# robustrobotics/multi_view_stereonet

Hardware: AMD Instinct MI355X
Metric: depthmaps/sec at 512x256, 64 hypotheses, 2 src views; L1 vs ref (higher is better)
Workload: dtype f32; 1 GPU; GTA-SfM-shaped 512x256, D=64 hypotheses, 2 source views, cost-volume filter + 5 refiners; global_batch=256, parallelism=dp1 (independent images, all-gather of metric rows)

## Files before the change

multi_view_stereonet_amd/csrc/mvsn_conv_wino.hip:

```cpp
#include <type_traits>
#include <utility>

#include "mvsn_resident.h"
#include "mvsn_conv_wino.h"

namespace mvsn {

constexpr int WN_THREADS = 512, WN_WAVES = 8;
constexpr int WN_TY = 16, WN_TX = 32;
constexpr int WN_WIDE_TY = 10, WN_WIDE_TX = 40, WN_WIDE_PC = WN_WIDE_TX / 2, WN_WIDE_NP = (WN_WIDE_TY / 2) * WN_WIDE_PC;
constexpr int WN_ROLL_PR = 6, WN_ROLL_NP = WN_ROLL_PR * WN_WIDE_PC, WN_ROLL_HY = 2 * WN_ROLL_PR + 3;
constexpr int WN_TILE_RP = 3;
constexpr int wn_pa(int dil) { return (dil + 3) / 4 * 4; }
constexpr int WN_UFLOATS = 16 * 128;
constexpr int WN_MAX_CHUNKS = 9;
constexpr int WN_LDS_MAX = 160 * 1024;

__device__ floatx4 g_wn_zero16 = {0.f, 0.f, 0.f, 0.f};

#ifndef MVSN_WN_ABLATE
#define MVSN_WN_ABLATE 0
#endif

#ifndef MVSN_RD_ABLATE
// ... 86 lines not shown
    {2, 4, 1, true, 0, 2, false, 24},
    {2, 3, 1, true, 1, 2, false, 24},
};
constexpr int WN_NFORMS = sizeof(WN_FORMS) / sizeof(WN_FORMS[0]);
constexpr int wn_find_form(const WinoForm &f, int from = 0) {
  for (int i = from; i < WN_NFORMS; ++i)
    if (WN_FORMS[i].same(f)) return i;
  return -1;
}
constexpr bool wn_forms_ok() {
  for (int i = 0; i < WN_NFORMS; ++i)
    if (WN_FORMS[i].bytes(WN_FORMS[i].chunks) > WN_LDS_MAX || wn_find_form(WN_FORMS[i], i + 1) >= 0) return false;
  return true;
}
static_assert(wn_forms_ok(), "a kernel form needs more than 160 KB of LDS, or is listed twice");

template <bool LDSONLY>
__device__ __forceinline__ void wn_barrier() {
  if constexpr (LDSONLY) asm volatile("s_waitcnt lgkmcnt(0)\n\ts_barrier" ::: "memory");
  else __syncthreads();
}

#pragma clang diagnostic push
#pragma clang diagnostic ignored "-Winline-asm"
template <bool ASM>
__device__ __forceinline__ void wn_dma16(const float *g, const float *l) {
  if constexpr (ASM) {
    const unsigned la = __builtin_amdgcn_readfirstlane((unsigned)(size_t)MVSN_LPTR(l));
    asm volatile("s_mov_b32 m0, %1\n\ts_nop 0\n\tglobal_load_lds_dwordx4 %0, off" ::"v"(g), "s"(la) : "memory", "m0");
  } else {
    __builtin_amdgcn_global_load_lds(MVSN_GPTR(g), MVSN_LPTR(l), 16, 0, 0);
  }
}
template <bool ASM>
__device__ __forceinline__ void wn_dma16_buf(const float *base, unsigned bytes, unsigned voff, const float *l) {
  if constexpr (ASM) {
    typedef int wn_srd_t __attribute__((ext_vector_type(4)));
    const size_t b = (size_t)base;
    wn_srd_t srd;
    srd[0] = __builtin_amdgcn_readfirstlane((int)(unsigned)b);
    srd[1] = __builtin_amdgcn_readfirstlane((int)((unsigned)(b >> 32) & 0xFFFFu));
    srd[2] = __builtin_amdgcn_readfirstlane((int)bytes);
    srd[3] = 0x00020000;
    const unsigned la = __builtin_amdgcn_readfirstlane((unsigned)(size_t)MVSN_LPTR(l));
#if MVSN_WN_NT_RAW
    asm volatile("s_mov_b32 m0, %2\n\ts_nop 0\n\tbuffer_load_dwordx4 %0, %1, 0 offen nt lds" ::"v"(voff), "s"(srd), "s"(la)
                 : "memory", "m0");
#else
    asm volatile("s_mov_b32 m0, %2\n\ts_nop 0\n\tbuffer_load_dwordx4 %0, %1, 0 offen lds" ::"v"(voff), "s"(srd), "s"(la)
                 : "memory", "m0");
#endif
  } else {
    __builtin_amdgcn_raw_ptr_buffer_load_lds(__builtin_amdgcn_make_buffer_rsrc(const_cast<float *>(base), 0, (int)bytes, 0x00020000),
                                             MVSN_LPTR(l), 16, (int)voff, 0, 0, MVSN_WN_NT_RAW ? 2 : 0);
  }
}
#pragma clang diagnostic pop

typedef unsigned wn_uintx2 __attribute__((ext_vector_type(2)));
typedef unsigned wn_uintx4 __attribute__((ext_vector_type(4)));
__device__ __forceinline__ __amdgpu_buffer_rsrc_t wn_rsrc(const void *base, unsigned bytes) {
  return __builtin_amdgcn_make_buffer_rsrc(const_cast<void *>(base), 0, (int)bytes, 0x00020000);
}
template <int AUX>
__device__ __forceinline__ void wn_store2(__amdgpu_buffer_rsrc_t r, unsigned voff, unsigned soff, float a, float b) {
  wn_uintx2 d;
  d[0] = __builtin_bit_cast(unsigned, a), d[1] = __builtin_bit_cast(unsigned, b);
  __builtin_amdgcn_raw_buffer_store_b64(d, r, (int)voff, (int)soff, AUX);
}
template <int AUX>
__device__ __forceinline__ void wn_store4(__amdgpu_buffer_rsrc_t r, unsigned voff, unsigned soff, floatx4 v) {
  __builtin_amdgcn_raw_buffer_store_b128(__builtin_bit_cast(wn_uintx4, v), r, (int)voff, (int)soff, AUX);
}

struct WinoDiv {
  unsigned mul, shift;
};
static WinoDiv wino_div(unsigned d) {
  unsigned s = 0;
  while ((1u << s) < d) ++s;
  const unsigned long long m = ((1ull << 32) * ((1ull << s) - d)) / d + 1;
  return WinoDiv{(unsigned)m, s};
}
__device__ __forceinline__ int wdiv(int n, WinoDiv f) { return (int)((__umulhi((unsigned)n, f.mul) + (unsigned)n) >> f.shift); }

struct WinoArgs {
  int n, cin, H, W, ntx, tiles, nchunks;
  WinoDiv fd_ntx;
  int cb0, cb1;
  const float *in1, *in2;
  size_t bs0, cs0;
  int rev;
  int D;
  int pr;
  WinoDiv fd_pr;
  int nty, rpy;
};

struct RideArgs {
  const float *x, *stats, *gamma, *beta;
  const float *res, *r_stats, *r_gamma, *r_beta;
  float *out;
  int units;
  WinoDiv fd_upp;
};
typedef const __attribute__((address_space(4))) float *wn_cfloat;
__device__ __forceinline__ float wn_sload(const float *p, size_t i) { return ((wn_cfloat)(size_t)p)[i]; }

__global__ void wino_pack_kernel(const float *__restrict__ w, int cin, int cout, int nchunks, int kd,
                                 float *__restrict__ out) {
  const int total = nchunks * WN_UFLOATS;
  const int idx = blockIdx.x * blockDim.x + threadIdx.x;
  if (idx >= total) return;
  const int lane = idx & 63, t = (idx >> 6) & 1, xi = (idx >> 7) & 15, chunk = idx >> 11;
  const int per_kz = nchunks / kd, kz = chunk / per_kz;
  const int co = t * 16 + (lane & 15), ci = (chunk - kz * per_kz) * 4 + (lane >> 4);
  float u = 0.0f;
  if (co < cout && ci < cin) {
    const float *g = w + (((size_t)co * cin + ci) * kd + kz) * 9;
    const float G[4][3] = {{1.f, 0.f, 0.f}, {0.5f, 0.5f, 0.5f}, {0.5f, -0.5f, 0.5f}, {0.f, 0.f, 1.f}};
    const int i = xi >> 2, j = xi & 3;
    for (int a = 0; a < 3; ++a)
      for (int b = 0; b < 3; ++b) u += G[i][a] * g[a * 3 + b] * G[j][b];
  }
  out[idx] = u;
}

#ifndef MVSN_WN_NO_FULLW
#define MVSN_WN_FULLW_OK 1
#else
#define MVSN_WN_FULLW_OK 0
#endif
template <int MODE, int KS, int NSTAGE, int DIL, bool VOL = false, int RIDE = 0, int TILE = 0, bool FULLW = false>
__global__ __launch_bounds__(WN_THREADS, 2) void conv_wino_kernel(WinoArgs g, const float *__restrict__ in,
                                                                  const float *__restrict__ upk,
                                                                  const float *__restrict__ bias,
                                                                  const float *__restrict__ in_stats,
                                                                  const float *__restrict__ in_gamma,
                                                                  const float *__restrict__ in_beta,
                                                                  float *__restrict__ out,
                                                                  float *__restrict__ out_partials, RideArgs rd,
                                                                  MVSN_VIS10) {
  extern __shared__ __attribute__((aligned(16))) float smem[];
#ifdef MVSN_WN_FORCE_DMA
  constexpr bool ASM_DMA = MVSN_WN_FORCE_DMA;
#else
  constexpr bool ASM_DMA = RIDE > 0 && DIL == 1;
#endif
#ifdef MVSN_WN_FORCE_BARRIER
  constexpr bool LDS_BARRIER = MVSN_WN_FORCE_BARRIER;
#else
  constexpr bool LDS_BARRIER = !VOL;
#endif
  constexpr bool RP = TILE == WN_TILE_RP;
  constexpr int WIDE = RP ? 0 : TILE;
  static_assert(!WIDE || (VOL && DIL == 1 && MVSN_WN_TRANSPOSED), "wide tiles: volume form only (transposed epilogue)");
  constexpr bool ROLL = WIDE == 2;
  constexpr int TY = ROLL ? 2 * WN_ROLL_PR : (WIDE ? WN_WIDE_TY : WN_TY), TX = WIDE ? WN_WIDE_TX : WN_TX;
  static_assert(!RP || (DIL > 1 && !VOL && !WIDE), "row-phase items: dilated 2-D layers");
  constexpr WinoForm L{KS, NSTAGE, DIL, VOL, RIDE, TILE, FULLW};
  constexpr int HY = L.hy(), XS = L.xs();
  constexpr int VS = RP ? 1 : DIL;
  constexpr int YS = RP ? DIL : 1;
  auto item_y0 = [](int tq) { return RP ? (tq & (DIL - 1)) + (int)((unsigned)tq / DIL) * (TY * DIL) : tq * TY; };
  constexpr int NP = ROLL ? WN_ROLL_NP : WN_WIDE_NP;
  constexpr int PA = wn_pa(DIL), DQ = XS / 4, GROUPS = HY * DQ, PIECES = (GROUPS + 63) / 64;
  static_assert(XS == TX + 2 * PA && HY == (ROLL ? WN_ROLL_HY : TY + 2 * VS), "the LDS plan's raw tile is this kernel's tile plus its halo");
  constexpr int RCST = L.rcst(), STAGE = L.stage();
  float *U = smem + L.u();
  static_assert(!FULLW || (DIL == 1 && WIDE == 0 && MVSN_WN_XF == 2 && MVSN_WN_TRANSPOSED), "full-width form: 16 x 32 tiles, burst + block");
  constexpr int SHIFT = (DIL == 1 && MVSN_WN_SHIFT && !FULLW) ? 1 : 0;
  constexpr int CSHIFT = (DIL > 1 && MVSN_WN_SHIFT) ? DIL : 0;
  constexpr int UST = KS * WN_UFLOATS;
  constexpr bool TR = DIL == 1 && MVSN_WN_TRANSPOSED;
  static_assert(!VOL || (KS == 2 && DIL == 1), "volume form: 32 channels in steps of 8, dilation 1");
  const int nsteps = (g.nchunks + KS - 1) / KS;
  const int uchunks = VOL ? NSTAGE * KS : nsteps * KS;

  const int tid = threadIdx.x, lane = tid & 63;
  const int wave = __builtin_amdgcn_readfirstlane(tid >> 6);
  const size_t plane = (size_t)g.H * g.W;
  const int ptiles = ROLL ? g.tiles : (RP ? DIL * g.rpy * g.ntx : g.D * g.tiles);
  auto roll_item = [&](int t, int &zA, int &prA0, int &sA) {
    const int R0 = t * WN_ROLL_PR;
    zA = wdiv(R0, g.fd_pr);
    prA0 = R0 - zA * g.pr;
    sA = g.pr - prA0 < WN_ROLL_PR ? g.pr - prA0 : WN_ROLL_PR;
  };
  const int total = g.n * ptiles;
  const int G = gridDim.x;
  const int slot = xcd_tile_index(blockIdx.x, G);
#ifdef MVSN_WN_STAMPS
  unsigned long long *dbg = (blockIdx.x == gridDim.x / 3 && tid == 0) ? g_wn_stamps : nullptr;
  unsigned long long *dbg_lds = reinterpret_cast<unsigned long long *>(U + L.stamps(uchunks));
  int dbg_i = 0;
  bool dbg_on = true;
#endif
  WN_STAMP();

  if constexpr (!VOL) {
    const int runs = g.nchunks * (WN_UFLOATS / 256);
    for (int run = wave; run < runs; run += WN_WAVES)
      wn_dma16<ASM_DMA>(upk + (size_t)run * 256 + lane * 4, U + run * 256);
    if (uchunks != g.nchunks)
      *reinterpret_cast<floatx4 *>(U + g.nchunks * WN_UFLOATS + tid * 4) = floatx4{0.f, 0.f, 0.f, 0.f};
  }

  float *bias_lds = U + L.bias(uchunks);
  if (tid < 32) bias_lds[tid] = bias ? bias[tid] : 0.0f;

  constexpr int STEP_PIECES = KS * 4 * PIECES;
  constexpr bool EVEN = STEP_PIECES % WN_WAVES == 0;
  constexpr int PER = EVEN ? STEP_PIECES / WN_WAVES : 2;
  static_assert(EVEN || (KS == 1 && PIECES == 3), "uneven DMA split only for the 12-piece case");
  static_assert(!EVEN || PIECES % PER == 0 || PER % PIECES == 0, "a wave's pieces stay within one channel");
  const int dch = EVEN ? (wave * PER) / PIECES : (wave & 3);
  const int dp0 = EVEN ? (wave * PER) % PIECES : (wave < 4 ? 0 : 2);
  const int dpn = EVEN ? (PER < PIECES ? PER : PIECES) : (wave < 4 ? 2 : 1);
  const float *zero = reinterpret_cast<const float *>(&g_wn_zero16);
  int pf_round = 0, pf_chunk = 0, pf_stage = 0;
  int pf_goff[PER];
  int pf_n = 0, pf_z = 0;
  bool pf_live = slot < total;
  int rd_young = 0;
  auto pf_plan = [&]() {
    const int flat = g.rev ? total - 1 - (pf_round * G + slot) : pf_round * G + slot;
    const int n = flat / ptiles;
    int tile = flat - n * ptiles;
    int r_pr0 = 0, r_s = WN_ROLL_PR;
    if constexpr (ROLL) {
      roll_item(tile, pf_z, r_pr0, r_s);
      tile = 0;
    } else if constexpr (VOL) {
      pf_z = tile / g.tiles;
      tile -= pf_z * g.tiles;
    }
    const int tyi = ROLL ? 0 : wdiv(tile, g.fd_ntx), txi = tile - tyi * g.ntx;
    const int y0 = ROLL ? 2 * r_pr0 : item_y0(tyi), x0 = txi * TX;
    pf_n = n;
    int lo;
    asm volatile("v_mbcnt_lo_u32_b32 %0, -1, 0\n\tv_mbcnt_hi_u32_b32 %0, -1, %0" : "=v"(lo));
#pragma unroll
    for (int i = 0; i < PER; ++i) {
      const int e = (dp0 + i) * 64 + lo;
      const int row = e / DQ, q = e - row * DQ;
      int gy = y0 - DIL + YS * row;
      const int gx = x0 - PA + 4 * q;
      int zsh = 0;
      if constexpr (ROLL) {
        const bool isb = (r_s < WN_ROLL_PR) & (row >= 2 * r_s + 1);
        gy = isb ? row - (2 * r_s + 2) : gy;
        zsh = isb ? g.H * g.W : 0;
      }
      const bool ok = (i < dpn) & (e < GROUPS) & (gy >= 0) & (gy < g.H) & (gx >= 0) & (gx < g.W);
      pf_goff[i] = ok ? (zsh + gy * g.W + gx) * (MVSN_WN_BUFDMA ? 4 : 1) : -1;
    }
  };
  auto pf_issue = [&]() {
    if (!pf_live) return;
    rd_young += PER;
    bool cok;
    const float *src;
    unsigned rbytes = 0;
    bool roll_first = false;
    if constexpr (ROLL) {
      const int kz = pf_chunk >> 2, c = (pf_chunk & 3) * 8 + dch, zz = pf_z + kz - 1;
      cok = zz >= 0 && zz < g.D;
      roll_first = zz < 0;
      const int zlo = zz < 0 ? 0 : zz, zhi = zz + 1 < g.D ? zz + 1 : g.D - 1;
      const int np = zhi - zlo + 1 > 0 ? zhi - zlo + 1 : 0;
      const int zsel = zlo < g.D - 1 ? zlo : g.D - 1;
      src = in + (size_t)(unsigned)__builtin_amdgcn_readfirstlane((pf_n * 32 + c) * g.D + zsel) * plane;
      rbytes = (unsigned)np * (unsigned)plane * 4u;
      rbytes = (unsigned)__builtin_amdgcn_readfirstlane((int)rbytes);
    } else if constexpr (VOL) {
      const int kz = pf_chunk >> 2, c = (pf_chunk & 3) * 8 + dch, zz = pf_z + kz - 1;
      cok = zz >= 0 && zz < g.D;
      src = in + (((size_t)pf_n * 32 + c) * g.D + (cok ? zz : 0)) * plane;
    } else {
      const int c = pf_chunk * (KS * 4) + dch;
      cok = c < g.cin;
      const int cc = cok ? c : 0, c1 = cc - g.cb0, c2 = c1 - g.cb1;
      src = c1 < 0 ? in + (size_t)pf_n * g.bs0 + (size_t)cc * g.cs0
          : c2 < 0 ? g.in1 + ((size_t)pf_n * g.cb1 + c1) * plane
                   : g.in2 + ((size_t)pf_n * (g.cin - g.cb0 - g.cb1) + c2) * plane;
    }
    float *dst = smem + pf_stage * STAGE + dch * RCST + SHIFT + CSHIFT * (dch & 1);
    const unsigned pbytes = ROLL ? rbytes : (cok ? (unsigned)plane * 4u : 0u);
#pragma unroll
    for (int i = 0; i < PER; ++i) {
      if (i < dpn) {
        if ((dp0 + i) * 64 + lane < GROUPS) {
          if constexpr (ROLL) {
            static_assert(!ROLL || MVSN_WN_BUFDMA, "rolling strips: descriptor DMA only");
            unsigned off = (unsigned)pf_goff[i];
            off -= roll_first ? (unsigned)plane * 4u : 0u;
            wn_dma16_buf<ASM_DMA>(src, pbytes, off, dst + (dp0 + i) * 256);
          } else if constexpr (MVSN_WN_BUFDMA) {
            wn_dma16_buf<ASM_DMA>(src, pbytes, (unsigned)pf_goff[i], dst + (dp0 + i) * 256);
          } else {
            const float *p = (cok && pf_goff[i] >= 0) ? src + pf_goff[i] : zero;
            wn_dma16<ASM_DMA>(p, dst + (dp0 + i) * 256);
          }
        }
      }
    }
// ... 107 lines not shown
            else xf_mask |= 1u << i;
          }
        }
      }
      int c = xf_chunk * (KS * 4) + dch;
      bool live = c < g.cin;
      if constexpr (VOL) {
        const int zz = z + (xf_chunk >> 2) - 1;
        c = (xf_chunk & 3) * 8 + dch;
        live = zz >= 0 && zz < g.D;
        if constexpr (ROLL) {
          const bool liveb = zz + 1 < g.D;
          xf_mask = (live ? xf_maska : 0u) | (liveb ? xf_maskb : 0u);
          live = live || liveb;
        }
      }
      if (live) {
        const float mean = in_stats[((size_t)n * 4 + (c >> 3)) * 2 + 0];
        const float rstd = in_stats[((size_t)n * 4 + (c >> 3)) * 2 + 1];
        xf_sc = rstd * in_gamma[c];
        xf_sh = in_beta[c] - mean * xf_sc;
      } else {
        xf_on = false;
      }
    }
  };
  auto xf_apply = [&]() {
    if constexpr (MODE == 1) {
      if (xf_on) {
        float *dst = smem + xf_stage * STAGE + dch * RCST + lane * 4 + SHIFT + CSHIFT * (dch & 1);
#pragma unroll
        for (int i = 0; i < PER; ++i)
          if ((xf_mask >> i) & 1u) {
            float *q = dst + (dp0 + i) * 256;
            if constexpr (SHIFT || CSHIFT % 4 != 0) {
              float e[4] = {q[0], q[1], q[2], q[3]};
#pragma unroll
              for (int r = 0; r < 4; ++r) e[r] = lrelu02(e[r] * xf_sc + xf_sh);
              q[0] = e[0], q[1] = e[1], q[2] = e[2], q[3] = e[3];
            } else {
              floatx4 v = *reinterpret_cast<floatx4 *>(q);
#pragma unroll
              for (int r = 0; r < 4; ++r) v[r] = lrelu02(v[r] * xf_sc + xf_sh);
              *reinterpret_cast<floatx4 *>(q) = v;
            }
          }
      }
      xf_stage = xf_stage + 1 == NSTAGE ? 0 : xf_stage + 1;
      if (++xf_chunk == nsteps) xf_chunk = 0, ++xf_round;
    }
  };

  int tr_round = 0, tr_chunk = 0, tr_stage = 0;
  auto tr_setup = [&]() {
    if constexpr (ROLL) {
      const int lin = tr_round * G + slot;
      if (lin < total) {
        const int flat = g.rev ? total - 1 - lin : lin;
        int zA, prA0, sA;
        roll_item(flat - (flat / ptiles) * ptiles, zA, prA0, sA);
        ya = 2 * lane_pr + (lane_pr >= sA ? 1 : 0);
      }
    }
  };
  auto dslot = [](int j) { return SHIFT ? j : (j & 1) * 2 + (j >> 1); };
  auto tr_load = [&](float (&d)[KS][4][4], int h0 = 0, int h1 = KS) {
#pragma unroll
    for (int h = 0; h < KS; ++h) {
      if (h < h0 || h >= h1) continue;
      const float *raw = smem + tr_stage * STAGE + (h * 4 + kc) * RCST + ya * XS + xa + (PA - DIL) + SHIFT + CSHIFT * (kc & 1);
      if constexpr (FULLW) {
        const float2 *r2 = reinterpret_cast<const float2 *>(raw + 1);
#pragma unroll
        for (int i = 0; i < 4; ++i) {
          const float2 c = r2[i * (XS / 2)];
          d[h][i][1] = c.x, d[h][i][2] = c.y;
        }
      } else if constexpr (SHIFT) {
        const float2 *r2 = reinterpret_cast<const float2 *>(raw);
#pragma unroll
        for (int i = 0; i < 4; ++i) {
          const float2 lo = r2[i * (XS / 2)], hi = r2[i * (XS / 2) + 1];
          d[h][i][0] = lo.x, d[h][i][1] = lo.y, d[h][i][2] = hi.x, d[h][i][3] = hi.y;
        }
      } else if constexpr (DIL == 1) {
        int oa = 0, ob = 1;
        asm volatile("" : "+v"(oa), "+v"(ob));
        const float *ra = raw + oa, *rb = raw + ob;
#pragma unroll
        for (int i = 0; i < 4; ++i) {
          d[h][i][0] = ra[i * XS], d[h][i][1] = ra[i * XS + 2];
          d[h][i][2] = rb[i * XS], d[h][i][3] = rb[i * XS + 2];
        }
      } else {
#pragma unroll
        for (int i = 0; i < 4; ++i) {
          d[h][i][0] = raw[i * VS * XS], d[h][i][1] = raw[i * VS * XS + 2 * DIL];
          d[h][i][2] = raw[i * VS * XS + DIL], d[h][i][3] = raw[i * VS * XS + 3 * DIL];
        }
      }
    }
  };
  auto tr_finish = [&](float (&d)[KS][4][4], float (&v)[KS][16], int h0 = 0, int h1 = KS) {
#pragma unroll
    for (int h = 0; h < KS; ++h) {
      if (h < h0 || h >= h1) continue;
      if constexpr (FULLW) {
        float t1[4], t2[4];
        {
          const float a0 = d[h][0][1], a1 = d[h][1][1], a2 = d[h][2][1], a3 = d[h][3][1];
          const float b0 = d[h][0][2], b1 = d[h][1][2], b2 = d[h][2][2], b3 = d[h][3][2];
          t1[0] = a0 - a2, t1[1] = a1 + a2, t1[2] = a2 - a1, t1[3] = a1 - a3;
          t2[0] = b0 - b2, t2[1] = b1 + b2, t2[2] = b2 - b1, t2[3] = b1 - b3;
        }
#pragma unroll
        for (int i = 0; i < 4; ++i) {
          v[h][i * 4 + 0] = dpp_mov<0x111>(t2[i]) - t2[i];
          v[h][i * 4 + 1] = t1[i] + t2[i];
          v[h][i * 4 + 2] = t2[i] - t1[i];
          v[h][i * 4 + 3] = t1[i] - dpp_mov<0x101>(t1[i]);
        }
        continue;
      }
      float t[4][4];
#pragma unroll
      for (int j = 0; j < 4; ++j) {
        const float d0 = d[h][0][dslot(j)], d1 = d[h][1][dslot(j)], d2 = d[h][2][dslot(j)], d3 = d[h][3][dslot(j)];
        t[0][j] = d0 - d2;
        t[1][j] = d1 + d2;
        t[2][j] = d2 - d1;
        t[3][j] = d1 - d3;
      }
#pragma unroll
      for (int i = 0; i < 4; ++i) {
        v[h][i * 4 + 0] = t[i][0] - t[i][2];
        v[h][i * 4 + 1] = t[i][1] + t[i][2];
        v[h][i * 4 + 2] = t[i][2] - t[i][1];
        v[h][i * 4 + 3] = t[i][1] - t[i][3];
      }
    }
  };
  auto tr_advance = [&]() {
    tr_stage = tr_stage + 1 == NSTAGE ? 0 : tr_stage + 1;
    if (++tr_chunk == nsteps) {
      tr_chunk = 0;
      ++tr_round;
      tr_setup();
    }
  };

  constexpr int RN = RIDE > 0 ? RIDE : 1;
  floatx4 rd_v[RN];
  float rd_sc = 0.f, rd_sh = 0.f, rd_rsc = 0.f, rd_rsh = 0.f;
  int rd_u = 0;
  bool rd_ok = false;
  float *rds = U + L.res(uchunks) + wave * (RN * 256);
  auto rd_issue = [&](int flat, int chunk) {
    if constexpr (RIDE > 0) {
      const int u = ((flat * nsteps + chunk) * WN_WAVES + wave) * RN;
      rd_ok = flat >= 0 && u < rd.units;
      rd_u = rd_ok ? u : 0;
      const int pl = wdiv(rd_u, rd.fd_upp), c = pl & 31, n = pl >> 5;
      const float mean = wn_sload(rd.stats, ((size_t)n * 4 + (c >> 3)) * 2 + 0);
      const float rstd = wn_sload(rd.stats, ((size_t)n * 4 + (c >> 3)) * 2 + 1);
      rd_sc = rstd * wn_sload(rd.gamma, c);
      rd_sh = wn_sload(rd.beta, c) - mean * rd_sc;
      rd_young = 0;
      const __amdgpu_buffer_rsrc_t xs = wn_rsrc(rd.x + (size_t)rd_u * 256, RN * 1024);
#pragma unroll
      for (int j = 0; j < RN; ++j)
        if (!(MVSN_RD_ABLATE & 1))
          rd_v[j] = __builtin_bit_cast(floatx4, __builtin_amdgcn_raw_buffer_load_b128(xs, lane * 16 + j * 1024, 0, 2));
      if (rd.res && !(MVSN_RD_ABLATE & 4)) {
#pragma unroll
        for (int j = 0; j < RN; ++j)
          wn_dma16_buf<ASM_DMA>(rd.res + (size_t)rd_u * 256, RN * 1024, (unsigned)(lane * 16 + j * 1024), rds + j * 256);
      }
      if (rd.r_stats) {
        const float rm = wn_sload(rd.r_stats, ((size_t)n * 4 + (c >> 3)) * 2 + 0);
        rd_rsc = wn_sload(rd.r_stats, ((size_t)n * 4 + (c >> 3)) * 2 + 1) * wn_sload(rd.r_gamma, c);
        rd_rsh = wn_sload(rd.r_beta, c) - rm * rd_rsc;
      }
    }
  };
  auto rd_consume = [&](int ln) {
    if constexpr (RIDE > 0) {
      floatx4 o[RN];
#pragma unroll
      for (int j = 0; j < RN; ++j) {
        if (MVSN_RD_ABLATE & 16) asm volatile("" ::"v"(rd_v[j]));
        if (MVSN_RD_ABLATE & 2) continue;
#pragma unroll
        for (int k = 0; k < 4; ++k) o[j][k] = lrelu02(rd_v[j][k] * rd_sc + rd_sh);
        if (rd.res) {
          const floatx4 r = *reinterpret_cast<const floatx4 *>(rds + j * 256 + ln * 4);
          if (rd.r_stats) {
#pragma unroll
            for (int k = 0; k < 4; ++k) o[j][k] += lrelu02(r[k] * rd_rsc + rd_rsh);
          } else {
#pragma unroll
            for (int k = 0; k < 4; ++k) o[j][k] += r[k];
          }
        }
      }
      if (rd_ok && !(MVSN_RD_ABLATE & 2)) {
        const __amdgpu_buffer_rsrc_t os = wn_rsrc(rd.out + (size_t)rd_u * 256, RN * 1024);
#pragma unroll
        for (int j = 0; j < RN; ++j) wn_store4<2>(os, (unsigned)(ln * 16 + j * 1024), 0, o[j]);
      }
    }
  };

  float v[KS][16];
  if (total_steps > 0) {
    tr_setup();
    xf_prepare();
    wait_landed(total_steps - 1 < NSTAGE - 1 ? total_steps - 1 : NSTAGE - 1);
    xf_apply();
    xf_prepare();
    wn_barrier<LDS_BARRIER>();
    float d0[KS][4][4];
    tr_load(d0);
    tr_finish(d0, v);
    tr_advance();
    rd_issue(-1, 0);
  }

  floatx4 acc[16][2];
  auto finish_tile = [&](int n, int z, int tile_id, int y0, int x0) {
    int lq;
    asm volatile("v_mbcnt_lo_u32_b32 %0, -1, 0\n\tv_mbcnt_hi_u32_b32 %0, -1, %0" : "=v"(lq));
    const int cl = lq & 15, gq = lq >> 4;
    constexpr int PSH = DIL <= 2 ? 1 : 0;
    auto slot_h = [](int r, int sec) { return PSH ? (r >> 1) : sec; };
    auto slot_k = [](int r, int sec) { return DIL == 1 ? 2 * (r & 1) + sec : (DIL == 2 ? (r & 1) + 2 * sec : r); };
    const int oy = y0 + (RP ? DIL : 1) * ya;
    const int xg0 = DIL == 8 ? 16 * (gq >> 1) + 4 * (gq & 1) : 8 * gq;
    const int xg1 = xg0 + (DIL == 8 ? 8 : 4);
    const bool row0 = oy < g.H, row1 = oy + DIL < g.H;
    const bool q0 = x0 + xg0 < g.W, q1 = x0 + xg1 < g.W;
    const size_t cstride = VOL ? (size_t)g.D * plane : plane;
    const __amdgpu_buffer_rsrc_t osrd = wn_rsrc(out + (size_t)n * 32 * cstride + (size_t)z * plane, (unsigned)(32 * cstride * 4));
    const unsigned obase = ((unsigned)cl * (unsigned)cstride + (unsigned)(oy * g.W + x0)) * 4u;
    const unsigned ovoff0 = q0 ? obase + (unsigned)xg0 * 4u : 0xFFFFFFFFu, ovoff1 = q1 ? obase + (unsigned)xg1 * 4u : 0xFFFFFFFFu;
    const int cnt = ((row0 ? 1 : 0) + (row1 ? 1 : 0)) * ((q0 ? 4 : 0) + (q1 ? 4 : 0));
    float s[2] = {0.f, 0.f};
    float y[2][2][8];
#pragma unroll
    for (int t = 0; t < 2; ++t) {
      const float bv = bias_lds[t * 16 + cl];
#pragma unroll
      for (int r = 0; r < 4; ++r) {
        float s0[4], s1[4];
#pragma unroll
        for (int j = 0; j < 4; ++j) {
          s0[j] = acc[j][t][r] + acc[4 + j][t][r] + acc[8 + j][t][r];
          s1[j] = acc[4 + j][t][r] - acc[8 + j][t][r] - acc[12 + j][t][r];
        }
        y[t][0][slot_h(r, 0) * 4 + slot_k(r, 0)] = s0[0] + s0[1] + s0[2] + bv;
        y[t][0][slot_h(r, 1) * 4 + slot_k(r, 1)] = s0[1] - s0[2] - s0[3] + bv;
        y[t][1][slot_h(r, 0) * 4 + slot_k(r, 0)] = s1[0] + s1[1] + s1[2] + bv;
        y[t][1][slot_h(r, 1) * 4 + slot_k(r, 1)] = s1[1] - s1[2] - s1[3] + bv;
      }
#pragma unroll
      for (int rr = 0; rr < 2; ++rr) {
        const bool rok = rr ? row1 : row0;
#pragma unroll
        for (int h = 0; h < 2; ++h) {
          const bool ok = rok && (h ? q1 : q0);
          if (rok && (!(MVSN_WN_ABLATE & 64) || n < 0))
            wn_store4<MVSN_WN_NT_STORES ? 2 : 0>(
                osrd, h ? ovoff1 : ovoff0, (unsigned)(((size_t)(t * 16) * cstride + (size_t)rr * DIL * g.W) * 4),
                floatx4{y[t][rr][4 * h], y[t][rr][4 * h + 1], y[t][rr][4 * h + 2], y[t][rr][4 * h + 3]});
          if (ok) {
#pragma unroll
            for (int k = 0; k < 4; ++k) s[t] += y[t][rr][4 * h + k];
          }
        }
      }
    }
    WN_STAMP();
    if (out_partials != nullptr) {
      auto sum8 = [](float v) {
        v += dpp_mov<0xB1>(v);
        v += dpp_mov<0x4E>(v);
        v += dpp_mov<0x141>(v);
        return v;
      };
      const int hi = (lq >> 3) & 1;
      const float npos = 8.0f * (float)cnt;
      const float rn = cnt == 16 ? 0.0078125f : (cnt == 8 ? 0.015625f : (cnt == 4 ? 0.03125f : 0.0f));
      float m[2], qv[2] = {0.f, 0.f};
#pragma unroll
      for (int t = 0; t < 2; ++t) {
        s[t] = sum8(s[t]);
        m[t] = s[t] * rn;
      }
#pragma unroll
      for (int t = 0; t < 2; ++t)
#pragma unroll
        for (int rr = 0; rr < 2; ++rr)
#pragma unroll
          for (int h = 0; h < 2; ++h)
            if ((rr ? row1 : row0) && (h ? q1 : q0)) {
#pragma unroll
              for (int k = 0; k < 4; ++k) {
                const float dv = y[t][rr][4 * h + k] - m[t];
                qv[t] += dv * dv;
              }
            }
#pragma unroll
      for (int t = 0; t < 2; ++t) qv[t] = sum8(qv[t]);
      int rtile = tile_id, rwave = wave;
      bool rec_ok = true;
      if constexpr (RP) {
        const int yq = oy & (TY - 1);
        rtile = (oy / TY) * g.ntx + x0 / TX, rwave = yq / (2 * DIL) * DIL + yq % DIL;
        rec_ok = oy < g.nty * TY;
      }
      if ((lq & 7) == 0 && rec_ok) {
        float *rec = out_partials + (((size_t)n * (RP ? g.tiles : ptiles) + (size_t)z * g.tiles + rtile) * WN_WAVES + rwave) * 48;
        rec += gq * 12 + hi * 3;
#pragma unroll
        for (int t = 0; t < 2; ++t) {
          rec[t * 6 + 0] = npos;
          rec[t * 6 + 1] = m[t];
          rec[t * 6 + 2] = qv[t];
        }
      }
    }
  };

  auto finish_tile_tr = [&](int n, int z, int tile_id, int y0, int x0, int r_s) {
    int lq;
    asm volatile("v_mbcnt_lo_u32_b32 %0, -1, 0\n\tv_mbcnt_hi_u32_b32 %0, -1, %0" : "=v"(lq));
    const int pc = lq & 15, gq = lq >> 4;
    int oy = y0 + 2 * wave, ox = x0 + 2 * pc;
    bool slot_ok = true;
    unsigned zb = 0;
    if constexpr (WIDE != 0) {
      const int q = wave * 16 + pc;
      slot_ok = q < NP;
      const int qq = slot_ok ? q : 0, pr = qq / WN_WIDE_PC;
      oy = y0 + 2 * pr, ox = x0 + 2 * (qq - pr * WN_WIDE_PC);
      if constexpr (ROLL) {
        const bool pb = pr >= r_s;
        oy = pb ? 2 * (pr - r_s) : oy;
        zb = pb ? (unsigned)plane : 0u;
        slot_ok = slot_ok & (!pb | (z + 1 < g.D));
      }
    }
    const bool row0 = oy < g.H, row1 = oy + 1 < g.H, cok = slot_ok && ox < g.W;
    const size_t cstride = VOL ? (size_t)g.D * plane : plane;
    const __amdgpu_buffer_rsrc_t osrd = wn_rsrc(out + (size_t)n * 32 * cstride + (size_t)z * plane, (unsigned)(32 * cstride * 4));
    const unsigned ovoff = cok ? ((unsigned)(4 * gq) * (unsigned)cstride + zb + (unsigned)(oy * g.W + ox)) * 4u : 0xFFFFFFFFu;
    const unsigned ovoff0 = (!WIDE || row0) ? ovoff : 0xFFFFFFFFu, ovoff1 = (!WIDE || row1) ? ovoff : 0xFFFFFFFFu;
    float s[2] = {0.f, 0.f};
    float y[2][4][4];
#pragma unroll
    for (int t = 0; t < 2; ++t) {
      const floatx4 bv = *reinterpret_cast<const floatx4 *>(bias_lds + t * 16 + 4 * gq);
#pragma unroll
      for (int r = 0; r < 4; ++r) {
        float s0[4], s1[4];
#pragma unroll
        for (int j = 0; j < 4; ++j) {
          s0[j] = acc[j][t][r] + acc[4 + j][t][r] + acc[8 + j][t][r];
          s1[j] = acc[4 + j][t][r] - acc[8 + j][t][r] - acc[12 + j][t][r];
        }
        y[t][r][0] = s0[0] + s0[1] + s0[2] + bv[r];
        y[t][r][1] = s0[1] - s0[2] - s0[3] + bv[r];
        y[t][r][2] = s1[0] + s1[1] + s1[2] + bv[r];
        y[t][r][3] = s1[1] - s1[2] - s1[3] + bv[r];
        if (!(MVSN_WN_ABLATE & 64) || n < 0) {
          const unsigned so = (unsigned)((size_t)(t * 16 + r) * cstride * 4);
          if (WIDE || row0) wn_store2<MVSN_WN_NT_TR ? 2 : 0>(osrd, ovoff0, so, y[t][r][0], y[t][r][1]);
          if (WIDE || row1) wn_store2<MVSN_WN_NT_TR ? 2 : 0>(osrd, ovoff1, so + (unsigned)g.W * 4u, y[t][r][2], y[t][r][3]);
        }
        if (row0 && cok) s[t] += y[t][r][0] + y[t][r][1];
        if (row1 && cok) s[t] += y[t][r][2] + y[t][r][3];
      }
    }
    WN_STAMP();
    if (out_partials != nullptr) {
      auto sum16 = [](float v) {
        v += dpp_mov<0xB1>(v);
        v += dpp_mov<0x4E>(v);
        v += dpp_mov<0x141>(v);
        v += dpp_mov<0x140>(v);
        return v;
      };
      const int vp = (g.W - x0) >> 1;
      float npos = (float)(8 * ((row0 ? 1 : 0) + (row1 ? 1 : 0)) * (vp > 16 ? 16 : vp));
      if constexpr (WIDE != 0)
        npos = sum16(cok ? (float)(8 * ((row0 ? 1 : 0) + (row1 ? 1 : 0))) : 0.0f);
      float m[2], qv[2] = {0.f, 0.f};
#pragma unroll
      for (int t = 0; t < 2; ++t) {
        s[t] = sum16(s[t]);
        m[t] = npos > 0.f ? s[t] / npos : 0.f;
      }
#pragma unroll
      for (int t = 0; t < 2; ++t)
#pragma unroll
        for (int r = 0; r < 4; ++r)
#pragma unroll
          for (int k = 0; k < 4; ++k)
            if ((k < 2 ? row0 : row1) && cok) {
              const float dv = y[t][r][k] - m[t];
              qv[t] += dv * dv;
            }
#pragma unroll
      for (int t = 0; t < 2; ++t) qv[t] = sum16(qv[t]);
      if (pc < 4) {
        float *rec = out_partials + (((size_t)n * ptiles + (ROLL ? (size_t)0 : (size_t)z * g.tiles) + tile_id) * WN_WAVES + wave) * 48;
        rec += gq * 12 + pc * 3;
        const int ga = gq >> 1;
        const bool a = pc == ga, b = pc == 2 + ga;
        rec[0] = (a || b) ? npos : 0.f;
        rec[1] = a ? m[0] : (b ? m[1] : 0.f);
        rec[2] = a ? qv[0] : (b ? qv[1] : 0.f);
      }
    }
  };

  int step = 0, mm_stage = 0;
  for (int round = 0; round < my_items; ++round) {
#ifdef MVSN_WN_STAMPS
    dbg_on = round >= 3 || my_items < 4;
#endif
    const int flat = g.rev ? total - 1 - (round * G + slot) : round * G + slot;
    const int n = flat / ptiles;
    int tile_id = flat - n * ptiles, z = 0;
    int r_pr0 = 0, r_s = WN_ROLL_PR;
    if constexpr (ROLL) {
      roll_item(tile_id, z, r_pr0, r_s);
    } else if constexpr (VOL) {
      z = tile_id / g.tiles;
      tile_id -= z * g.tiles;
    }
    const int tyi = ROLL ? 0 : wdiv(tile_id, g.fd_ntx), txi = ROLL ? 0 : tile_id - tyi * g.ntx;
    const int y0 = ROLL ? 2 * r_pr0 : item_y0(tyi), x0 = txi * TX;

#pragma unroll
    for (int xi = 0; xi < 16; ++xi) asm volatile("" : "=v"(acc[xi][0]), "=v"(acc[xi][1]));

    int chunk = 0;
    auto do_step = [&](auto firstc) {
      const bool has_next = step + 1 < total_steps;
      bool waited = false;
      if constexpr (RIDE > 0) {
        if (rd_young == PERV) asm volatile("s_waitcnt vmcnt(%0)" ::"n"(PERV) : "memory");
        else if (rd_young == PER) asm volatile("s_waitcnt vmcnt(%0)" ::"n"(PER) : "memory");
        else if (VOL && rd_young == 2) asm volatile("s_waitcnt vmcnt(2)" ::: "memory");
        else asm volatile("s_waitcnt vmcnt(0)" ::: "memory");
        rd_consume(lane);
        waited = true;
      }
      if (has_next) {
        const int rest = total_steps - (step + 2);
        if (!waited) wait_landed(rest < 0 ? 0 : (rest < NSTAGE - 2 ? rest : NSTAGE - 2));
        xf_apply();
        WN_STAMP();
        if (!(MVSN_WN_ABLATE & 8)) wn_barrier<LDS_BARRIER>();
        if (MVSN_WN_STAGGER > 0 && wave >= 4) __builtin_amdgcn_s_sleep(MVSN_WN_STAGGER);
        WN_STAMP();
        xf_prepare();
      }
      rd_issue(flat, chunk);
      float dn[KS][4][4];
      if (has_next && !(MVSN_WN_ABLATE & 32)) {
        if (MVSN_WN_XF == 1) tr_load(dn);
        else if (MVSN_WN_XF == 0) tr_load(dn, 0, 1);
      }
      auto multiply = [&](auto first, auto hc) {
        constexpr bool FIRST = decltype(first)::value;
        constexpr int h = decltype(hc)::value;
        const float *ub = U + (VOL ? mm_stage : chunk) * UST + h * WN_UFLOATS + lane;
        float fb[2][2];
        fb[0][0] = ub[0], fb[0][1] = ub[64];
        auto tcol = [&](int i, int j) {
          const float d0 = dn[h][0][dslot(j)], d1 = dn[h][1][dslot(j)], d2 = dn[h][2][dslot(j)], d3 = dn[h][3][dslot(j)];
          return i == 0 ? d0 - d2 : (i == 1 ? d1 + d2 : (i == 2 ? d2 - d1 : d1 - d3));
        };
        constexpr bool INTER = MVSN_WN_XF == 1 || (MVSN_WN_XF == 0 && h == 0);
        float tc[4], tn[4];
        if constexpr (INTER) {
#pragma unroll
          for (int j = 0; j < 4; ++j) tc[j] = tcol(0, j);
        } else {
          if (has_next && !(MVSN_WN_ABLATE & 32)) tr_load(dn, h, h + 1);
        }
#pragma unroll
        for (int xi = 0; xi < 16; ++xi) {
          const int cur = xi & 1, ti = xi >> 2, tj = xi & 3;
          if (INTER && ti < 3) tn[tj] = tcol(ti + 1, tj);
          if (xi + 1 < 16 && !(MVSN_WN_ABLATE & 2)) {
            fb[cur ^ 1][0] = ub[(xi + 1) * 128];
            fb[cur ^ 1][1] = ub[(xi + 1) * 128 + 64];
          }
          if constexpr (FIRST) {
            acc[xi][0] = TR ? mfma16x16x4(fb[cur][0], v[h][xi], floatx4{0.f, 0.f, 0.f, 0.f})
                            : mfma16x16x4(v[h][xi], fb[cur][0], floatx4{0.f, 0.f, 0.f, 0.f});
            acc[xi][1] = TR ? mfma16x16x4(fb[cur][1], v[h][xi], floatx4{0.f, 0.f, 0.f, 0.f})
                            : mfma16x16x4(v[h][xi], fb[cur][1], floatx4{0.f, 0.f, 0.f, 0.f});
          } else {
            acc[xi][0] = TR ? mfma16x16x4(fb[cur][0], v[h][xi], acc[xi][0]) : mfma16x16x4(v[h][xi], fb[cur][0], acc[xi][0]);
            acc[xi][1] = TR ? mfma16x16x4(fb[cur][1], v[h][xi], acc[xi][1]) : mfma16x16x4(v[h][xi], fb[cur][1], acc[xi][1]);
          }
          if (h == 0 && xi == 1 && has_next && !(MVSN_WN_ABLATE & 4)) {
            pf_issue();
            uq_issue();
          }
          if constexpr (INTER) {
            if (!(MVSN_WN_ABLATE & 1)) {
              v[h][xi] = tj == 0 ? tc[0] - tc[2] : (tj == 1 ? tc[1] + tc[2] : (tj == 2 ? tc[2] - tc[1] : tc[1] - tc[3]));
              if (MVSN_WN_PIN) asm volatile("" : "+v"(v[h][xi]));
            }
            if (tj == 3) {
#pragma unroll
              for (int k = 0; k < 4; ++k) tc[k] = tn[k];
            }
          }
          __builtin_amdgcn_sched_barrier(0);
        }
        if constexpr (!INTER) {
          if (!(MVSN_WN_ABLATE & 1)) {
            tr_finish(dn, v, h, h + 1);
#pragma unroll
            for (int xi = 0; xi < 16; ++xi)
              if (MVSN_WN_PIN) asm volatile("" : "+v"(v[h][xi]));
          }
          __builtin_amdgcn_sched_barrier(0);
        }
      };
      multiply(firstc, std::integral_constant<int, 0>{});
      if constexpr (KS == 2) multiply(std::false_type{}, std::integral_constant<int, 1>{});
      tr_advance();
      if constexpr (VOL) mm_stage = mm_stage + 1 == NSTAGE ? 0 : mm_stage + 1;
      WN_STAMP();
      ++step;
    };
    do_step(std::true_type{});
    for (chunk = 1; chunk < nsteps; ++chunk) do_step(std::false_type{});
    if (!(MVSN_WN_ABLATE & 16) || n < 0) {
      if constexpr (TR) finish_tile_tr(n, z, tile_id, y0, x0, r_s);
      else finish_tile(n, z, tile_id, y0, x0);
    }
  }
  if constexpr (RIDE > 0) {
    if (total_steps > 0) {
      asm volatile("s_waitcnt vmcnt(0)" ::: "memory");
      int ln;
      asm volatile("v_mbcnt_lo_u32_b32 %0, -1, 0\n\tv_mbcnt_hi_u32_b32 %0, -1, %0" : "=v"(ln));
      rd_consume(ln);
    }
  }
#ifdef MVSN_WN_STAMPS
  if (dbg)
    for (int i = 0; i < dbg_i; ++i) dbg[i] = dbg_lds[i];
#endif
}

constexpr int S2_TY = 16, S2_TX = 32;
constexpr int S2_ROWS = 2 * S2_TY + 3, S2_XS = 2 * S2_TX + 8, S2_DQ = S2_XS / 4;
constexpr int S2_GROUPS = S2_ROWS * S2_DQ, S2_PIECES = (S2_GROUPS + 63) / 64;
constexpr int S2_RCST = S2_ROWS * S2_XS + 1;
constexpr int S2_STAGE = 4 * S2_RCST;
constexpr int S2_UST = 4 * WN_UFLOATS;
constexpr int S2_STEPS = 8;
constexpr size_t S2_LDS_BYTES = (size_t)(2 * S2_STAGE + 2 * S2_UST + 32) * sizeof(float);
static_assert(S2_PIECES * 4 % WN_WAVES == 0, "a step's raw pieces divide evenly among the waves");
static_assert(S2_LDS_BYTES <= 160 * 1024, "LDS plan");

__global__ void wino_s2_pack_kernel(const float *__restrict__ w, float *__restrict__ out) {
  const int idx = blockIdx.x * blockDim.x + threadIdx.x;
  if (idx >= S2_STEPS * S2_UST) return;
  const int lane = idx & 63, t = (idx >> 6) & 1, xi = (idx >> 7) & 15, ph = (idx >> 11) & 3, cc = idx >> 13;
  const int py = ph >> 1, px = ph & 1;
  const int co = t * 16 + (lane & 15), ci = cc * 4 + (lane >> 4);
  const float *g = w + ((size_t)co * 32 + ci) * 25;
  const float G[4][3] = {{1.f, 0.f, 0.f}, {0.5f, 0.5f, 0.5f}, {0.5f, -0.5f, 0.5f}, {0.f, 0.f, 1.f}};
  const int i = xi >> 2, j = xi & 3;
  float u = 0.0f;
  for (int a = 0; a < 3; ++a)
    for (int b = 0; b < 3; ++b) {
      const int ky = 2 * a + py, kx = 2 * b + px;
      if (ky < 5 && kx < 5) u += G[i][a] * g[ky * 5 + kx] * G[j][b];
    }
  out[idx] = u;
}

#ifndef MVSN_S2_PIN
#define MVSN_S2_PIN 1
#endif
#ifndef MVSN_S2_CNTWAIT
#define MVSN_S2_CNTWAIT 1
#endif
struct WinoS2Args {
  int n, H, W, Ho, Wo, ntx, tiles;
  WinoDiv fd_ntx;
};

__global__ __launch_bounds__(WN_THREADS, 2) void conv_wino_s2_kernel(WinoS2Args g, const float *__restrict__ in,
                                                                     const float *__restrict__ upk,
// ... 370 lines not shown
```

multi_view_stereonet_amd/multi_view_stereonet.py:

```python
import ctypes
import threading
import warnings
from typing import Dict, List, Optional

import torch
import torch.nn as nn

from . import _native
from .params import REFINER_DILATIONS, build_parameter_tree

ListTensor = List[torch.Tensor]


class _Conv:

    def __init__(self, lib, weight: torch.Tensor, bias: Optional[torch.Tensor], stride: int = 1, dilation: int = 1):
        self.lib = lib
        self.cout, self.cin = int(weight.shape[0]), int(weight.shape[1])
        self.dims = weight.dim() - 2
        k = tuple(int(s) for s in weight.shape[2:])
        self.kd, self.kh, self.kw = (k if self.dims == 3 else (1,) + k)
        self.stride, self.dilation = stride, dilation
        self.bias = bias.detach().contiguous().float() if bias is not None else None
        self.weight = weight.detach().contiguous().float() if self.cout == 1 else None
        d = self.desc(1, 1 if self.dims == 2 else 2, 8, 32)
        n = lib.mvsn_conv_packed_floats(ctypes.byref(d))
        if n == 0:
            raise RuntimeError("mvsn_conv_packed_floats rejected the descriptor")
        self.packed = torch.empty(n, dtype=torch.float32, device=weight.device)
        w = weight.detach().contiguous().float()
        _native.check(lib.mvsn_conv_pack_weights(ctypes.byref(d), _native.ptr(w), _native.ptr(self.packed),
                                                 _native.stream()), "mvsn_conv_pack_weights")
        self.packed_bx = None
        dbx = self.desc(1, 1 if self.dims == 2 else 2, 8, 32, _native.CONV_BF16X3)
        if lib.mvsn_conv_bf16x3_supported(ctypes.byref(dbx)):
            nbx = lib.mvsn_conv_packed_floats(ctypes.byref(dbx))
            self.packed_bx = torch.empty(nbx, dtype=torch.float32, device=weight.device)
            _native.check(lib.mvsn_conv_pack_weights(ctypes.byref(dbx), _native.ptr(w), _native.ptr(self.packed_bx),
                                                     _native.stream()), "mvsn_conv_pack_weights(bf16x3)")

        self.packed_wino = None
        dwn = self.desc(1, 1, 8, 32, _native.CONV_FP32_WINO)
        if lib.mvsn_conv_winograd_supported(ctypes.byref(dwn)):
            nwn = lib.mvsn_conv_packed_floats(ctypes.byref(dwn))
            self.packed_wino = torch.empty(nwn, dtype=torch.float32, device=weight.device)
            _native.check(lib.mvsn_conv_pack_weights(ctypes.byref(dwn), _native.ptr(w), _native.ptr(self.packed_wino),
                                                     _native.stream()), "mvsn_conv_pack_weights(winograd)")

    def desc(self, n, depth, rows, cols, precision=_native.CONV_FP32):
        return _native.ConvDesc(n, self.cin, self.cout, depth, rows, cols, self.kd, self.kh, self.kw,
                                self.stride, self.dilation, precision)


class _Norm:
    def __init__(self, p):
        self.gamma = p.weight.detach().contiguous().float()
        self.beta = p.bias.detach().contiguous().float()


class EngineOptions:

    def __init__(self):
        self.fold_residual_blocks = False
        self.conv_precision = "fp32"
        self.winograd = True
        self.winograd_with_input_transform = True
        self.winograd_volume = True
        self.winograd_stride2 = True
        self.volume_materialise = True
        self.trim_tower_ends = True
        self.lazy_stats_max_samples = 8
        self.lazy_stats_max_records = 2048
        self.split_finalize = True
        self.cat_free_heads = True
        self.chain_form = "auto"
        self.carry_passes = True
        self.carry_min_bytes = 32 << 20
        self.carry_alternate = True
        self.carry_volume_passes = False
        self.towers = True
        self.plan_max_chains = 16
        self.plan_graph = True
        self.plan_max_bytes = 8 << 30
        self.banded_repair = True
        self.confidence = False

    NAMES = ("split_finalize", "banded_repair", "towers", "plan_max_chains", "plan_graph", "plan_max_bytes", "carry_passes", "carry_min_bytes", "carry_volume_passes", "carry_alternate", "chain_form", "fold_residual_blocks", "conv_precision", "winograd", "winograd_with_input_transform",
             "winograd_volume", "winograd_stride2", "volume_materialise", "trim_tower_ends", "cat_free_heads", "lazy_stats_max_samples",
             "lazy_stats_max_records", "confidence")


class _Records:
    __slots__ = ("partials", "tiles")

    def __init__(self, partials: torch.Tensor):
        self.partials, self.tiles = partials, int(partials.shape[1])


def _stats_arg(st):
    return (_native.ptr(st.partials), st.tiles) if isinstance(st, _Records) else (_native.ptr(st), 0)


class _Job:

    def __init__(self, r, stats, norm, residual=None, r_stats=None, r_norm=None):
        self.keep = (r, stats, norm, residual, r_stats, r_norm)
        n, spatial = r.shape[0], r[0, 0].numel()
        P = _native.ptr
        self.job = _native.ApplyJob(P(r), P(stats), P(norm.gamma), P(norm.beta), P(residual), P(r_stats),
                                    P(r_norm.gamma) if r_norm else None, P(r_norm.beta) if r_norm else None,
                                    P(r), n, 0, spatial)
        self.nbytes = 4.0 * r.numel() * (2 if residual is None else 3)

    def run_alone(self, eng):
        r, stats, norm, residual, r_stats, r_norm = self.keep
        if r_stats is not None:
            eng.gn_lrelu_add2(r, stats, norm, residual, r_stats, r_norm, out=r)
        else:
            eng.gn_lrelu(r, stats, norm, residual=residual, out=r)


class _SharedState:

    def __init__(self):
        self.words = None
        self.words_np = None
        self.seen = 0
        self.banded_latched = False
        self.warned = False
        self.clean = 0
        self.latch_forwards = self.LATCH_FORWARDS
        self.relatches = 0

    LATCH_FORWARDS = 256
    LATCH_CAP = 1 << 16

    def tick(self):
        if self.banded_latched:
            self.clean += 1
            if self.clean >= self.latch_forwards:
                self.banded_latched, self.clean = False, 0

    def rearm(self):
        self.banded_latched, self.warned, self.clean, self.latch_forwards, self.relatches = False, False, 0, self.LATCH_FORWARDS, 0

    def status_ptr(self) -> int:
        if self.words is None:
            self.words = torch.zeros(4, dtype=torch.int32).pin_memory()
            self.words_np = self.words.numpy()
        return self.words.data_ptr()

    def poll(self) -> int:
        if self.words_np is None:
            return 0
        count = int(self.words_np[1])
        fresh, self.seen = count - self.seen, count
        if fresh:
            if self.relatches:
                self.latch_forwards = min(self.latch_forwards * 2, self.LATCH_CAP)
            self.relatches += 1
            self.banded_latched, self.clean = True, 0
            if not self.warned:
                self.warned = True
                warnings.warn(
                    "mvsn_incremental_cost_volume(banded): an inter-workgroup hand-off timed out (status %d) -- the chain's "
                    "workgroups were not co-resident: the device is shared with other work.  That forward's chain was "
                    "recomputed in-stream by the single-launch form (its outputs are valid); this module no longer "
                    "chooses the banded form (net.reset_device_status() re-enables it)." % int(self.words_np[0]),
                    RuntimeWarning, stacklevel=3)
        return fresh


class ForwardPlan:

    def __init__(self):
        self.calls, self.keep = [], []
        self.replayable = True
        self.static_inputs: List[torch.Tensor] = []
        self.outputs: Optional[dict] = None
        self.graph = None
        self.uses = 0
        self.nbytes = 0
        self.chain_info = (None, None, None)

    def replay(self):
        stream = _native.stream()
        for fn, args, name in self.calls:
            rc = fn(*args, stream)
            if rc != 0:
                _native.check(rc, name)


class PlaneSweepEngine:

    def __getattr__(self, name):
        if name in EngineOptions.NAMES:
            return getattr(self.__dict__["opt"], name)
        raise AttributeError(name)

    def __setattr__(self, name, value):
        if name in EngineOptions.NAMES:
            setattr(self.__dict__["opt"], name, value)
        else:
            object.__setattr__(self, name, value)


    def __init__(self, net: "MultiViewStereoNet"):
        self.lib = lib = _native.load()
        self.carried_jobs = 0
        self.bf16_layers = 0
        self.banded_ok = True
        self.net_state = net.__dict__.setdefault("_shared_state", _SharedState())
        self.last_chain_form, self.last_chain_workspace, self.last_chain_shape = None, None, None
        self.last_cost_dtype = torch.float32
        self.recording: Optional["ForwardPlan"] = None
        self.plans: Dict[tuple, Optional[ForwardPlan]] = {}
        self.replays = 0
        self._carried_before = {}
        object.__setattr__(self, "opt", net.options)
        self.timeline: Optional[list] = None
        self.level_tag = ""
        fe = net.left_feature_extractor
        self.fe_down = [_Conv(lib, getattr(fe, f"conv{i}").weight, None, stride=2) for i in range(4)]
        self.fe_res = [(_Conv(lib, getattr(fe, f"res{i}").conv1.weight, None), _Norm(getattr(fe, f"res{i}").bn1))
                       for i in range(6)]
        self.fe_final = _Conv(lib, fe.conv_final.weight, fe.conv_final.bias)

        r = net.right_feature_extractor.refiner
        dev = r.conv0.weight.device
        self.refiner_packed = torch.empty(lib.mvsn_feature_refiner_packed_floats(), dtype=torch.float32, device=dev)
        tensors = [r.conv0.weight, r.conv0.bias, r.bn0.weight, r.bn0.bias, r.res0.conv1.weight, r.res0.conv1.bias,
                   r.res0.bn1.weight, r.res0.bn1.bias, r.conv_final.weight, r.conv_final.bias]
# ... 1062 lines not shown
```

Before: 3806 depthmaps/s.

## Carry volume normalize passes inside Winograd volume convs via hidden asm loads

Enables carrying the normalize+activation pass of volume layers inside the Winograd volume convolution kernel. The carried loads are issued as inline-asm nontemporal buffer loads that the compiler cannot see, and waits are counted manually alongside the DMA pieces. The residual path is dropped for the volume form, and the scale/shift computation is deferred to consume time. The goal is to remove a separate memory-bound elementwise pass over the large cost volume, at the cost of more register pressure and fragile manual vmcnt accounting.

```diff
diff --git a/multi_view_stereonet_amd/csrc/mvsn_conv_wino.hip b/multi_view_stereonet_amd/csrc/mvsn_conv_wino.hip
--- a/multi_view_stereonet_amd/csrc/mvsn_conv_wino.hip
+++ b/multi_view_stereonet_amd/csrc/mvsn_conv_wino.hip
@@ -262,6 +262,8 @@
 #else
   constexpr bool LDS_BARRIER = !VOL;
 #endif
+  constexpr bool ASM_RIDE = RIDE > 0 && VOL;
+  static_assert(!ASM_RIDE || ASM_DMA, "hidden carried loads: only next to hidden DMA pieces (the counted waits are the only ones)");
   constexpr bool RP = TILE == WN_TILE_RP;
   constexpr int WIDE = RP ? 0 : TILE;
   static_assert(!WIDE || (VOL && DIL == 1 && MVSN_WN_TRANSPOSED), "wide tiles: volume form only (transposed epilogue)");
@@ -675,6 +677,8 @@
   constexpr int RN = RIDE > 0 ? RIDE : 1;
   floatx4 rd_v[RN];
   float rd_sc = 0.f, rd_sh = 0.f, rd_rsc = 0.f, rd_rsh = 0.f;
+  float rd_mean = 0.f, rd_rstd = 0.f, rd_gamma = 0.f, rd_beta = 0.f;
+  constexpr bool RD_RES = !VOL;
   int rd_u = 0;
   bool rd_ok = false;
   float *rds = U + L.res(uchunks) + wave * (RN * 256);
@@ -684,22 +688,44 @@
       rd_ok = flat >= 0 && u < rd.units;
       rd_u = rd_ok ? u : 0;
       const int pl = wdiv(rd_u, rd.fd_upp), c = pl & 31, n = pl >> 5;
-      const float mean = wn_sload(rd.stats, ((size_t)n * 4 + (c >> 3)) * 2 + 0);
-      const float rstd = wn_sload(rd.stats, ((size_t)n * 4 + (c >> 3)) * 2 + 1);
-      rd_sc = rstd * wn_sload(rd.gamma, c);
-      rd_sh = wn_sload(rd.beta, c) - mean * rd_sc;
+      if constexpr (ASM_RIDE) {
+        rd_mean = wn_sload(rd.stats, ((size_t)n * 4 + (c >> 3)) * 2 + 0);
+        rd_rstd = wn_sload(rd.stats, ((size_t)n * 4 + (c >> 3)) * 2 + 1);
+        rd_gamma = wn_sload(rd.gamma, c);
+        rd_beta = wn_sload(rd.beta, c);
+      } else {
+        const float mean = wn_sload(rd.stats, ((size_t)n * 4 + (c >> 3)) * 2 + 0);
+        const float rstd = wn_sload(rd.stats, ((size_t)n * 4 + (c >> 3)) * 2 + 1);
+        rd_sc = rstd * wn_sload(rd.gamma, c);
+        rd_sh = wn_sload(rd.beta, c) - mean * rd_sc;
+      }
       rd_young = 0;
-      const __amdgpu_buffer_rsrc_t xs = wn_rsrc(rd.x + (size_t)rd_u * 256, RN * 1024);
-#pragma unroll
-      for (int j = 0; j < RN; ++j)
-        if (!(MVSN_RD_ABLATE & 1))
-          rd_v[j] = __builtin_bit_cast(floatx4, __builtin_amdgcn_raw_buffer_load_b128(xs, lane * 16 + j * 1024, 0, 2));
-      if (rd.res && !(MVSN_RD_ABLATE & 4)) {
+      if constexpr (ASM_RIDE) {
+        typedef int wn_srd_t __attribute__((ext_vector_type(4)));
+        const size_t b = (size_t)(rd.x + (size_t)rd_u * 256);
+        wn_srd_t srd;
+        srd[0] = __builtin_amdgcn_readfirstlane((int)(unsigned)b);
+        srd[1] = __builtin_amdgcn_readfirstlane((int)((unsigned)(b >> 32) & 0xFFFFu));
+        srd[2] = RN * 1024;
+        srd[3] = 0x00020000;
+        const unsigned voff = (unsigned)lane * 16u;
+#pragma unroll
+        for (int j = 0; j < RN; ++j)
+          if (rd_ok && !(MVSN_RD_ABLATE & 1))
+            asm volatile("buffer_load_dwordx4 %0, %1, %2, 0 offen offset:%3 nt" : "=v"(rd_v[j]) : "v"(voff), "s"(srd), "n"(j * 1024) : "memory");
+      } else {
+        const __amdgpu_buffer_rsrc_t xs = wn_rsrc(rd.x + (size_t)rd_u * 256, RN * 1024);
+#pragma unroll
+        for (int j = 0; j < RN; ++j)
+          if (!(MVSN_RD_ABLATE & 1))
+            rd_v[j] = __builtin_bit_cast(floatx4, __builtin_amdgcn_raw_buffer_load_b128(xs, lane * 16 + j * 1024, 0, 2));
+      }
+      if (RD_RES && rd.res && !(MVSN_RD_ABLATE & 4)) {
 #pragma unroll
         for (int j = 0; j < RN; ++j)
           wn_dma16_buf<ASM_DMA>(rd.res + (size_t)rd_u * 256, RN * 1024, (unsigned)(lane * 16 + j * 1024), rds + j * 256);
       }
-      if (rd.r_stats) {
+      if (RD_RES && rd.r_stats) {
         const float rm = wn_sload(rd.r_stats, ((size_t)n * 4 + (c >> 3)) * 2 + 0);
         rd_rsc = wn_sload(rd.r_stats, ((size_t)n * 4 + (c >> 3)) * 2 + 1) * wn_sload(rd.r_gamma, c);
         rd_rsh = wn_sload(rd.r_beta, c) - rm * rd_rsc;
@@ -709,15 +735,23 @@
   auto rd_consume = [&](int ln) {
     if constexpr (RIDE > 0) {
       floatx4 o[RN];
+      if constexpr (ASM_RIDE) {
+        if (!rd_ok) return;
+#pragma unroll
+        for (int j = 0; j < RN; ++j)
+          if (!(MVSN_RD_ABLATE & 1)) asm volatile("" : "+v"(rd_v[j]));
+        rd_sc = rd_rstd * rd_gamma;
+        rd_sh = rd_beta - rd_mean * rd_sc;
+      }
 #pragma unroll
       for (int j = 0; j < RN; ++j) {
         if (MVSN_RD_ABLATE & 16) asm volatile("" ::"v"(rd_v[j]));
         if (MVSN_RD_ABLATE & 2) continue;
 #pragma unroll
         for (int k = 0; k < 4; ++k) o[j][k] = lrelu02(rd_v[j][k] * rd_sc + rd_sh);
-        if (rd.res) {
+        if (RD_RES && rd.res) {
           const floatx4 r = *reinterpret_cast<const floatx4 *>(rds + j * 256 + ln * 4);
-          if (rd.r_stats) {
+          if (RD_RES && rd.r_stats) {
 #pragma unroll
             for (int k = 0; k < 4; ++k) o[j][k] += lrelu02(r[k] * rd_rsc + rd_rsh);
           } else {
@@ -973,7 +1007,10 @@
       const bool has_next = step + 1 < total_steps;
       bool waited = false;
       if constexpr (RIDE > 0) {
-        if (rd_young == PERV) asm volatile("s_waitcnt vmcnt(%0)" ::"n"(PERV) : "memory");
+        if constexpr (ASM_RIDE) {
+          if (rd_young != PERV) asm volatile("s_waitcnt vmcnt(0)" ::: "memory");
+          asm volatile("s_waitcnt vmcnt(%0)" ::"n"(PERV) : "memory");
+        } else if (rd_young == PERV) asm volatile("s_waitcnt vmcnt(%0)" ::"n"(PERV) : "memory");
         else if (rd_young == PER) asm volatile("s_waitcnt vmcnt(%0)" ::"n"(PER) : "memory");
         else if (VOL && rd_young == 2) asm volatile("s_waitcnt vmcnt(2)" ::: "memory");
         else asm volatile("s_waitcnt vmcnt(0)" ::: "memory");
diff --git a/multi_view_stereonet_amd/multi_view_stereonet.py b/multi_view_stereonet_amd/multi_view_stereonet.py
--- a/multi_view_stereonet_amd/multi_view_stereonet.py
+++ b/multi_view_stereonet_amd/multi_view_stereonet.py
@@ -77,7 +77,7 @@
         self.carry_passes = True
         self.carry_min_bytes = 32 << 20
         self.carry_alternate = True
-        self.carry_volume_passes = False
+        self.carry_volume_passes = True
         self.towers = True
         self.plan_max_chains = 16
         self.plan_graph = True
```

After: 3882 depthmaps/s (median of 6 runs). 1.02x the previous value.
